# TheProParadox/3dspa_code

Measured on AMD Instinct MI355X. Metric: train-step tracks/sec (B x N_tracks) at T=150, C=772, higher is better.
Workload: dtype bf16

## Files before the change

### 3dspa_code_amd/csrc/rows.hip

```cpp
#include <algorithm>

#include "common.hpp"

namespace SPA_NS {

void k_zero(spa3d_ctx* c, void* p, int64_t bytes) {
  if (c->dry || bytes == 0) return;
  hipError_t e = hipMemsetAsync(p, 0, (size_t)bytes, c->stream);
  if (e != hipSuccess && !c->hip_err) { c->hip_err = (int)e; c->err = std::string("hipMemsetAsync: ") + hipGetErrorString(e); }
}
struct I32x32 { int32_t v[32]; };
__global__ void set_i32_kernel(int32_t* __restrict__ dst, I32x32 a, int n) {
  const int t = threadIdx.x;
#pragma unroll
  for (int i = 0; i < 32; ++i) if (t == i && i < n) dst[i] = a.v[i];
}
void k_set_i32(spa3d_ctx* c, int32_t* dst, const int32_t* host, int64_t n) {
  if (c->dry) return;
  for (int64_t i0 = 0; i0 < n; i0 += 32) {
    I32x32 a; const int m = (int)std::min<int64_t>(32, n - i0);
    for (int i = 0; i < 32; ++i) a.v[i] = i < m ? host[i0 + i] : 0;
    set_i32_kernel<<<1, 64, 0, c->stream>>>(dst + i0, a, m);
  }
  SPA_LAUNCH_CHECK(c);
}
__global__ void mul_kernel(float* __restrict__ a, const float* __restrict__ b, int64_t n) {
  for (int64_t i = (int64_t)blockIdx.x * 256 + threadIdx.x; i < n; i += (int64_t)gridDim.x * 256) a[i] *= b[i];
}
void k_mul(spa3d_ctx* c, float* a, const float* b, int64_t n) {
  if (c->dry || n == 0) return;
  mul_kernel<<<GRID1D(n, 256), 256, 0, c->stream>>>(a, b, n); SPA_LAUNCH_CHECK(c);
}
template <typename T>
__global__ void cast_from_f32_kernel(const float* __restrict__ s, T* __restrict__ d, int64_t n) {
  for (int64_t i = (int64_t)blockIdx.x * 256 + threadIdx.x; i < n; i += (int64_t)gridDim.x * 256) st(d + i, s[i]);
}
template <typename T> void k_cast_from_f32(spa3d_ctx* c, const float* s, T* d, int64_t n) {
  if (c->dry || n == 0) return;
  cast_from_f32_kernel<T><<<GRID1D(n, 256), 256, 0, c->stream>>>(s, d, n); SPA_LAUNCH_CHECK(c);
}
template <typename T>
__global__ void cast_to_f32_kernel(const T* __restrict__ s, float* __restrict__ d, int64_t n) {
  for (int64_t i = (int64_t)blockIdx.x * 256 + threadIdx.x; i < n; i += (int64_t)gridDim.x * 256) d[i] = ld(s + i);
}
template <typename T> void k_cast_to_f32(spa3d_ctx* c, const T* s, float* d, int64_t n) {
  if (c->dry || n == 0) return;
  cast_to_f32_kernel<T><<<GRID1D(n, 256), 256, 0, c->stream>>>(s, d, n); SPA_LAUNCH_CHECK(c);
}
template <typename T>
__global__ void colsum_kernel(const T* __restrict__ x, int64_t rows, int n, int64_t ld_, float* __restrict__ out, int64_t rows_per_block,
                              int rgroup, int rskip, const DetCfg* det) {
  __shared__ float red[4][64];
  const int col = blockIdx.x * 64 + (threadIdx.x & 63), w = threadIdx.x >> 6;
  int64_t r0 = (int64_t)blockIdx.y * rows_per_block, r1 = std::min<int64_t>(rows, r0 + rows_per_block);
  float s = 0.f;
  if (col < n) for (int64_t r = r0 + w; r < r1; r += 4) {
    int64_t pr = r; if (rgroup > 0) pr = r + (r / rgroup + 1) * (int64_t)rskip;
    s += ld(x + pr * ld_ + col);
  }
  red[w][threadIdx.x & 63] = s;
  __syncthreads();
  if (w == 0 && col < n) grad_add(det_read(det), out + col, red[0][threadIdx.x] + red[1][threadIdx.x] + red[2][threadIdx.x] + red[3][threadIdx.x]);
}
template <typename T>
__global__ __launch_bounds__(256) void colsum_vec_kernel(const T* __restrict__ x, int64_t rows, int n, int64_t ld_, float* __restrict__ out,
                                                         int64_t rows_per_block, int rgroup, int rskip, const DetCfg* det) {
  constexpr int NV = VecOf<T>::N;
  __shared__ float red[8][32 * NV];
  const int cx = threadIdx.x & 31, ry = threadIdx.x >> 5;
  const int ch = blockIdx.x * 32 + cx;
  const int64_t r0 = (int64_t)blockIdx.y * rows_per_block, r1 = std::min<int64_t>(rows, r0 + rows_per_block);
  float a[NV];
#pragma unroll
  for (int j = 0; j < NV; ++j) a[j] = 0.f;
  if (ch * NV < n)
    for (int64_t r = r0 + ry; r < r1; r += 8) {
      int64_t pr = r; if (rgroup > 0) pr = r + (r / rgroup + 1) * (int64_t)rskip;
      float v[NV]; load_vec<T, NV>(x + pr * ld_ + ch * NV, v);
#pragma unroll
      for (int j = 0; j < NV; ++j) a[j] += v[j];
    }
#pragma unroll
  for (int j = 0; j < NV; ++j) red[ry][cx * NV + j] = a[j];
  __syncthreads();
  if (ry == 0 && ch * NV < n)
#pragma unroll
    for (int j = 0; j < NV; ++j) {
      float s_ = 0.f;
#pragma unroll
      for (int k = 0; k < 8; ++k) s_ += red[k][cx * NV + j];
      grad_add(det_read(det), out + ch * NV + j, s_);
    }
}
template <typename T>
void k_colsum(spa3d_ctx* c, const T* x, int64_t rows, int n, int64_t ld_, float* out, int rgroup, int rskip) {
  if (c->dry || rows == 0) return;
  constexpr int NV = VecOf<T>::N;
  if (n % NV == 0 && ld_ % NV == 0 && (((uintptr_t)x) & 15) == 0) {
    const int64_t gx = cdiv(n / NV, 32);
    int64_t sp = std::max<int64_t>(1, std::min<int64_t>(cdiv(rows, 64), 2048 / gx + 1));
    int64_t rpb_ = cdiv(rows, sp);
    colsum_vec_kernel<T><<<dim3((unsigned)gx, (unsigned)cdiv(rows, rpb_)), 256, 0, c->stream>>>(x, rows, n, ld_, out, rpb_, rgroup, rskip, c->det);
    SPA_LAUNCH_CHECK(c);
    return;
  }
  int64_t splits = std::max<int64_t>(1, std::min<int64_t>(cdiv(rows, 256), 1024 / std::max<int64_t>(1, cdiv(n, 64)) + 1));
  int64_t rpb = cdiv(rows, splits);
  colsum_kernel<T><<<dim3((unsigned)cdiv(n, 64), (unsigned)cdiv(rows, rpb)), 256, 0, c->stream>>>(x, rows, n, ld_, out, rpb, rgroup, rskip, c->det);
  SPA_LAUNCH_CHECK(c);
}

template <typename T>
__global__ void gather_rows_kernel(const T* __restrict__ src, int64_t srows, T* __restrict__ dst, int64_t n, int d) {
  const int64_t tot = n * d;
  for (int64_t i = (int64_t)blockIdx.x * 256 + threadIdx.x; i < tot; i += (int64_t)gridDim.x * 256) {
    int64_t r = i / d; int j = (int)(i - r * d);
    dst[i] = src[r * srows * d + j];
  }
}
template <typename T> void k_gather_rows(spa3d_ctx* c, const T* src, int64_t srows, T* dst, int64_t n, int d) {
  if (c->dry || n == 0) return;
  gather_rows_kernel<T><<<GRID1D(n * d, 256), 256, 0, c->stream>>>(src, srows, dst, n, d); SPA_LAUNCH_CHECK(c);
}
template <typename T, int MODE>
__global__ void rows_idx_kernel(const T* __restrict__ src, const int32_t* __restrict__ idx, T* __restrict__ dst, int64_t n, int d) {
  constexpr int NV = VecOf<T>::N;
  const int cpr = d / NV;
  const int64_t tot = n * cpr;
  for (int64_t i = (int64_t)blockIdx.x * 256 + threadIdx.x; i < tot; i += (int64_t)gridDim.x * 256) {
    const int64_t r = i / cpr; const int ch = (int)(i - r * cpr);
    const int64_t other = idx[r];
    const int64_t so = (MODE == 0 ? other : r) * d + ch * NV, dofs = (MODE == 0 ? r : other) * d + ch * NV;
    if constexpr (MODE == 2) {
      float a[NV], b[NV];
      load_vec<T, NV>(src + so, a); load_vec<T, NV>(dst + dofs, b);
#pragma unroll
      for (int j = 0; j < NV; ++j) b[j] += a[j];
      store_vec<T, NV>(dst + dofs, b);
    } else {
      *(uint4*)(dst + dofs) = *(const uint4*)(src + so);
    }
  }
}
template <typename T> void k_rows_idx(spa3d_ctx* c, int mode, const T* src, const int32_t* idx, T* dst, int64_t n, int d) {
  if (c->dry || n == 0) return;
  constexpr int NV = VecOf<T>::N;
  if (d % NV) { if (!c->hip_err) { c->hip_err = -5; c->err = "rows_idx: row width must be a multiple of 16 bytes"; } return; }
  const dim3 g = GRID1D(n * (d / NV), 256);
  if (mode == 0) rows_idx_kernel<T, 0><<<g, 256, 0, c->stream>>>(src, idx, dst, n, d);
  else if (mode == 1) rows_idx_kernel<T, 1><<<g, 256, 0, c->stream>>>(src, idx, dst, n, d);
  else rows_idx_kernel<T, 2><<<g, 256, 0, c->stream>>>(src, idx, dst, n, d);
  SPA_LAUNCH_CHECK(c);
}
template <typename T>
__global__ void add_rows_strided_kernel(T* __restrict__ dst, const T* __restrict__ src, int64_t drows, int64_t n, int d) {
  const int64_t tot = n * d;
  for (int64_t i = (int64_t)blockIdx.x * 256 + threadIdx.x; i < tot; i += (int64_t)gridDim.x * 256) {
    int64_t r = i / d; int j = (int)(i - r * d);
    T* p = dst + r * drows * d + j;
    st(p, ld(p) + ld(src + i));
  }
}
template <typename T> void k_add_rows_strided(spa3d_ctx* c, T* dst, const T* src, int64_t drows, int64_t n, int d) {
  if (c->dry || n == 0) return;
  add_rows_strided_kernel<T><<<GRID1D(n * d, 256), 256, 0, c->stream>>>(dst, src, drows, n, d); SPA_LAUNCH_CHECK(c);
}

__global__ __launch_bounds__(256) void prune_count_kernel(const float* __restrict__ km, int64_t nseq, int S, int32_t* __restrict__ cnt) {
  const int lane = threadIdx.x & 63;
  for (int64_t seq = (int64_t)blockIdx.x * 4 + (threadIdx.x >> 6); seq < nseq; seq += (int64_t)gridDim.x * 4) {
    int n = 0;
    for (int t = lane; t < S; t += 64) n += km[seq * S + t] != 0.f ? 1 : 0;
#pragma unroll
    for (int o = 32; o > 0; o >>= 1) n += __shfl_xor(n, o, 64);
    if (lane == 0) cnt[seq] = n;
  }
}
__global__ __launch_bounds__(1024) void prune_scan_kernel(const int32_t* __restrict__ cnt, int64_t n, int32_t* __restrict__ off) {
  __shared__ int32_t part[1024];
  const int tid = threadIdx.x;
  const int64_t per = (n + 1023) / 1024, a = tid * per, b = a + per < n ? a + per : n;
  int32_t s = 0;
  for (int64_t i = a; i < b; ++i) s += cnt[i];
  part[tid] = s;
  __syncthreads();
  for (int o = 1; o < 1024; o <<= 1) {
    const int32_t v = tid >= o ? part[tid - o] : 0;
    __syncthreads();
    part[tid] += v;
    __syncthreads();
  }
  int32_t run = tid ? part[tid - 1] : 0;
  for (int64_t i = a; i < b; ++i) { off[i] = run; run += cnt[i]; }
  if (tid == 1023) off[n] = part[1023];
}
__global__ __launch_bounds__(256) void prune_fill_kernel(const float* __restrict__ km, int64_t nseq, int S, const int32_t* __restrict__ off,
                                                         int32_t* __restrict__ row_src) {
  const int lane = threadIdx.x & 63;
  for (int64_t seq = (int64_t)blockIdx.x * 4 + (threadIdx.x >> 6); seq < nseq; seq += (int64_t)gridDim.x * 4) {
    int base = off[seq];
    for (int t0 = 0; t0 < S; t0 += 64) {
      const int t = t0 + lane;
      const bool keep = t < S && km[seq * S + t] != 0.f;
      const unsigned long long m = __ballot(keep);
      if (keep) row_src[base + __popcll(m & ((1ull << lane) - 1ull))] = (int32_t)(seq * S + t);
      base += __popcll(m);
    }
  }
}
int64_t k_prune_plan(spa3d_ctx* c, const float* km, int64_t nseq, int S, int32_t* cnt, int32_t* seq_off, int32_t* row_src) {
  if (c->dry) return nseq * S;
  prune_count_kernel<<<(unsigned)std::min<int64_t>(cdiv(nseq, 4), 8192), 256, 0, c->stream>>>(km, nseq, S, cnt); SPA_LAUNCH_CHECK(c);
  prune_scan_kernel<<<1, 1024, 0, c->stream>>>(cnt, nseq, seq_off); SPA_LAUNCH_CHECK(c);
  prune_fill_kernel<<<(unsigned)std::min<int64_t>(cdiv(nseq, 4), 8192), 256, 0, c->stream>>>(km, nseq, S, seq_off, row_src); SPA_LAUNCH_CHECK(c);
  int32_t kept = 0;
  if (hipMemcpyAsync(&kept, seq_off + nseq, sizeof(int32_t), hipMemcpyDeviceToHost, c->stream) != hipSuccess ||
      hipStreamSynchronize(c->stream) != hipSuccess) {
    if (!c->hip_err) { c->hip_err = -4; c->err = "prune plan: reading the kept-row count failed"; }
    return nseq * S;
  }
  return kept;
}

__global__ __launch_bounds__(256) void share_plan_kernel(const int32_t* __restrict__ qframe, int Q, int32_t* __restrict__ slot, int32_t* __restrict__ nslot_b,
                                                         int32_t* __restrict__ first_q) {
  extern __shared__ int32_t sh[];
  const int b = blockIdx.x;
  const int32_t* fr = qframe + (int64_t)b * Q;
  for (int q = threadIdx.x; q < Q; q += 256) {
    const int32_t f = fr[q];
    int first = q;
    for (int p = 0; p < q; ++p) if (fr[p] == f) { first = p; break; }
    sh[q] = first;
  }
  __syncthreads();
  if (threadIdx.x == 0) {
    int n = 0;
    for (int q = 0; q < Q; ++q) {
      if (sh[q] == q) { first_q[(int64_t)b * Q + n] = q; sh[q] = -(n + 1); ++n; }
    }
    nslot_b[b] = n;
  }
  __syncthreads();
  for (int q = threadIdx.x; q < Q; q += 256) {
    const int32_t v = sh[q];
    slot[(int64_t)b * Q + q] = v < 0 ? -v - 1 : -sh[v] - 1;
  }
}
__global__ __launch_bounds__(256) void share_plan_finish_kernel(const int32_t* __restrict__ qframe, int B, int Q, int32_t* __restrict__ slot,
                                                                const int32_t* __restrict__ nslot_b, const int32_t* __restrict__ first_q,
                                                                int32_t* __restrict__ slot_b, int32_t* __restrict__ slot_f, int32_t* __restrict__ slot_q0,
                                                                int32_t* __restrict__ total) {
  __shared__ int32_t off[1025];
  if (threadIdx.x == 0) { int a = 0; for (int b = 0; b < B; ++b) { off[b] = a; a += nslot_b[b]; } off[B] = a; total[0] = a; }
  __syncthreads();
  for (int64_t i = threadIdx.x; i < (int64_t)B * Q; i += 256) {
    const int b = (int)(i / Q), j = (int)(i - (int64_t)b * Q);
    slot[i] += off[b];
    if (j < nslot_b[b]) { slot_b[off[b] + j] = b; slot_f[off[b] + j] = qframe[(int64_t)b * Q + first_q[i]]; slot_q0[off[b] + j] = b * Q + first_q[i]; }
  }
}
int64_t k_share_plan(spa3d_ctx* c, const int32_t* qframe, int64_t B, int Q, int32_t* slot, int32_t* slot_b, int32_t* slot_f, int32_t* slot_q0,
                     int32_t* scratch ) {
  if (c->dry) return B * Q;
  if (B > 1024 || Q > 12288) return B * Q;
  int32_t* first_q = scratch; int32_t* nslot_b = scratch + B * Q; int32_t* total = nslot_b + B;
  share_plan_kernel<<<(unsigned)B, 256, Q * sizeof(int32_t), c->stream>>>(qframe, Q, slot, nslot_b, first_q); SPA_LAUNCH_CHECK(c);
  share_plan_finish_kernel<<<1, 256, 0, c->stream>>>(qframe, (int)B, Q, slot, nslot_b, first_q, slot_b, slot_f, slot_q0, total); SPA_LAUNCH_CHECK(c);
  int32_t n = 0;
  if (hipMemcpyAsync(&n, total, sizeof(int32_t), hipMemcpyDeviceToHost, c->stream) != hipSuccess || hipStreamSynchronize(c->stream) != hipSuccess) {
    if (!c->hip_err) { c->hip_err = -4; c->err = "share plan: reading the slot count failed"; }
    return B * Q;
  }
  return n;
}
template <typename T>
__global__ void share_assemble_kernel(const T* __restrict__ qtok, const T* __restrict__ lat, const int32_t* __restrict__ slot_b,
                                      const int32_t* __restrict__ slot_f, int64_t nslot, int64_t BQ, int L, int Cl, int D, T* __restrict__ xU) {
  constexpr int NV = VecOf<T>::N;
  const int cpr = D / NV;
  const int64_t nlat = nslot * L, tot = (nlat + BQ) * cpr;
  for (int64_t i = (int64_t)blockIdx.x * 256 + threadIdx.x; i < tot; i += (int64_t)gridDim.x * 256) {
    const int64_t row = i / cpr; const int j = (int)(i - row * cpr) * NV;
    float v[NV];
    if (row >= nlat) load_vec<T, NV>(qtok + (row - nlat) * D + j, v);
    else {
      const int64_t s_ = row / L; const int n = (int)(row - s_ * L);
      const T* lr = lat + ((int64_t)slot_b[s_] * L + n) * Cl;
      if (j < Cl) load_vec<T, NV>(lr + j, v);
      else {
        const int base = j - Cl + 5 * slot_f[s_];
#pragma unroll
        for (int e = 0; e < NV; ++e) { const int cc = base + e; v[e] = (cc >= 0 && cc < Cl) ? ld(lr + cc) : 0.f; }
      }
    }
    store_vec<T, NV>(xU + row * D + j, v);
  }
}
template <typename T>
void k_share_assemble(spa3d_ctx* c, const T* qtok, const T* lat, const int32_t* slot_b, const int32_t* slot_f, int64_t nslot, int64_t BQ, int L, int Cl,
                      int D, T* xU) {
  if (c->dry || BQ == 0) return;
  constexpr int NV = VecOf<T>::N;
  if (D % NV || Cl % NV) { if (!c->hip_err) { c->hip_err = -5; c->err = "share assemble: widths must be multiples of 16 bytes"; } return; }
  share_assemble_kernel<T><<<GRID1D((nslot * L + BQ) * (D / NV), 256), 256, 0, c->stream>>>(qtok, lat, slot_b, slot_f, nslot, BQ, L, Cl, D, xU);
  SPA_LAUNCH_CHECK(c);
}
template <typename T, bool ADD>
__global__ void share_expand_kernel(const T* __restrict__ src, const int32_t* __restrict__ slot, const int32_t* __restrict__ slot_q0, int64_t nslot,
                                    int64_t nseq, int S, int d, const T* add, T* dst) {
  constexpr int NV = VecOf<T>::N;
  const int cpr = d / NV, L = S - 1;
  const int64_t tot = nseq * S * cpr;
  for (int64_t i = (int64_t)blockIdx.x * 256 + threadIdx.x; i < tot; i += (int64_t)gridDim.x * 256) {
    const int64_t row = i / cpr; const int ch = (int)(i - row * cpr);
    const int64_t seq = row / S; const int tkn = (int)(row - seq * S);
    const int32_t sl = slot[seq];
    const int64_t sr = tkn == 0 ? nslot * L + seq : (int64_t)sl * L + tkn - 1;
    if constexpr (ADD) {
      float b[NV];
      load_vec<T, NV>(add + row * d + ch * NV, b);
      if (tkn == 0 || slot_q0[sl] == (int32_t)seq) {
        float a[NV];
        load_vec<T, NV>(src + sr * d + ch * NV, a);
#pragma unroll
        for (int j = 0; j < NV; ++j) b[j] += a[j];
      }
      store_vec<T, NV>(dst + row * d + ch * NV, b);
    } else {
      *(uint4*)(dst + row * d + ch * NV) = *(const uint4*)(src + sr * d + ch * NV);
    }
  }
}
template <typename T>
void k_share_expand(spa3d_ctx* c, const T* src, const int32_t* slot, const int32_t* slot_q0, int64_t nslot, int64_t nseq, int S, int d, const T* add, T* dst) {
  if (c->dry || nseq == 0) return;
  constexpr int NV = VecOf<T>::N;
  if (d % NV) { if (!c->hip_err) { c->hip_err = -5; c->err = "share expand: row width must be a multiple of 16 bytes"; } return; }
  const dim3 g = GRID1D(nseq * S * (d / NV), 256);
  if (add) share_expand_kernel<T, true><<<g, 256, 0, c->stream>>>(src, slot, slot_q0, nslot, nseq, S, d, add, dst);
  else share_expand_kernel<T, false><<<g, 256, 0, c->stream>>>(src, slot, slot_q0, nslot, nseq, S, d, nullptr, dst);
  SPA_LAUNCH_CHECK(c);
}
template <typename T>
__global__ __launch_bounds__(256) void share_reduce_kernel(const T* __restrict__ src, const int32_t* __restrict__ slot, const int32_t* __restrict__ slot_b,
                                                           int64_t nslot, int Q, int S, int d, T* __restrict__ dstU) {
  constexpr int NV = VecOf<T>::N;
  extern __shared__ int32_t members[];
  __shared__ int32_t wcnt[4], nmem;
  const int64_t s_ = blockIdx.x; const int L = S - 1, cpr = d / NV;
  const int b = slot_b[s_];
  const int lane = threadIdx.x & 63, wv = threadIdx.x >> 6;
  int base = 0;
  for (int q0 = 0; q0 < Q; q0 += 256) {
    const int q = q0 + threadIdx.x;
    const bool mine = q < Q && slot[(int64_t)b * Q + q] == (int32_t)s_;
    const unsigned long long m = __ballot(mine);
    if (lane == 0) wcnt[wv] = __popcll(m);
    __syncthreads();
    int pre = base;
    for (int w2 = 0; w2 < wv; ++w2) pre += wcnt[w2];
    if (mine) members[pre + __popcll(m & ((1ull << lane) - 1ull))] = q;
    base += wcnt[0] + wcnt[1] + wcnt[2] + wcnt[3];
    __syncthreads();
  }
  if (threadIdx.x == 0) nmem = base;
  __syncthreads();
  const int nm = nmem;
  for (int i = threadIdx.x; i < L * cpr; i += 256) {
    const int n = i / cpr, ch = i - n * cpr;
    float acc[NV];
#pragma unroll
    for (int j = 0; j < NV; ++j) acc[j] = 0.f;
    for (int m = 0; m < nm; ++m) {
      float v[NV];
      load_vec<T, NV>(src + (((int64_t)b * Q + members[m]) * S + 1 + n) * d + ch * NV, v);
#pragma unroll
      for (int j = 0; j < NV; ++j) acc[j] += v[j];
    }
    store_vec<T, NV>(dstU + (s_ * L + n) * d + ch * NV, acc);
  }
}
template <typename T>
void k_share_reduce(spa3d_ctx* c, const T* src, const int32_t* slot, const int32_t* slot_b, int64_t nslot, int64_t nseq, int Q, int S, int d, T* dstU) {
  if (c->dry || nseq == 0) return;
  constexpr int NV = VecOf<T>::N;
  if (d % NV) { if (!c->hip_err) { c->hip_err = -5; c->err = "share reduce: row width must be a multiple of 16 bytes"; } return; }
  if (nslot > 0) share_reduce_kernel<T><<<(unsigned)nslot, 256, Q * sizeof(int32_t), c->stream>>>(src, slot, slot_b, nslot, Q, S, d, dstU);
  SPA_LAUNCH_CHECK(c);
  k_gather_rows<T>(c, src, S, dstU + nslot * (S - 1) * d, nseq, d);
}

template <typename T>
__global__ void assemble_kernel(const T* __restrict__ qtok, const T* __restrict__ lat, const int32_t* __restrict__ qframe, int64_t BQ, int Q,
                                int L, int Cl, int D, T* __restrict__ seq) {
  const int64_t tot = BQ * (L + 1) * D;
  for (int64_t i = (int64_t)blockIdx.x * 256 + threadIdx.x; i < tot; i += (int64_t)gridDim.x * 256) {
    int64_t row = i / D; int j = (int)(i - row * D);
    int64_t bq = row / (L + 1); int tkn = (int)(row - bq * (L + 1));
    T v;
    if (tkn == 0) v = qtok[bq * D + j];
    else {
      int64_t b = bq / Q; int n = tkn - 1;
      const T* lr = lat + (b * L + n) * Cl;
      if (j < Cl) v = lr[j];
      else {
        int64_t cc = (int64_t)(j - Cl) + 5 * (int64_t)qframe[bq];
        if (cc >= 0 && cc < Cl) v = lr[cc]; else { T z; st(&z, 0.f); v = z; }
      }
    }
    seq[i] = v;
  }
}
template <typename T>
__global__ void assemble_vec_kernel(const T* __restrict__ qtok, const T* __restrict__ lat, const int32_t* __restrict__ qframe, unsigned nchunk,
                                    int Q, int L, int Cl, int D, T* __restrict__ seq) {
  constexpr int NV = VecOf<T>::N;
  const unsigned cpr = (unsigned)D / NV;
  for (unsigned i = blockIdx.x * 256u + threadIdx.x; i < nchunk; i += gridDim.x * 256u) {
    const unsigned row = i / cpr; const int j = (int)(i - row * cpr) * NV;
    const unsigned bq = row / (unsigned)(L + 1); const int tkn = (int)(row - bq * (unsigned)(L + 1));
    float v[NV];
    if (tkn == 0) load_vec<T, NV>(qtok + (int64_t)bq * D + j, v);
    else {
      const unsigned b = bq / (unsigned)Q;
      const T* lr = lat + ((int64_t)b * L + (tkn - 1)) * Cl;
      if (j < Cl) load_vec<T, NV>(lr + j, v);
      else {
        const int base = j - Cl + 5 * qframe[bq];
#pragma unroll
        for (int e = 0; e < NV; ++e) { const int cc = base + e; v[e] = (cc >= 0 && cc < Cl) ? ld(lr + cc) : 0.f; }
      }
    }
    store_vec<T, NV>(seq + (int64_t)row * D + j, v);
  }
}
template <typename T>
void k_assemble_readout(spa3d_ctx* c, const T* qtok, const T* lat, const int32_t* qframe, int64_t B, int Q, int L, int Cl, int D, T* seq) {
  if (c->dry || B == 0) return;
  constexpr int NV = VecOf<T>::N;
  const int64_t nchunk = B * Q * (L + 1) * (D / NV);
  if (D % NV == 0 && Cl % NV == 0 && nchunk < 0x7fffffffLL && ((((uintptr_t)qtok) | ((uintptr_t)lat) | ((uintptr_t)seq)) & 15) == 0) {
    assemble_vec_kernel<T><<<GRID1D(nchunk, 256), 256, 0, c->stream>>>(qtok, lat, qframe, (unsigned)nchunk, Q, L, Cl, D, seq);
  } else {
    assemble_kernel<T><<<GRID1D(B * Q * (L + 1) * D, 256), 256, 0, c->stream>>>(qtok, lat, qframe, B * Q, Q, L, Cl, D, seq);
  }
  SPA_LAUNCH_CHECK(c);
}
template <typename T, bool ACC>
__global__ void assemble_bwd_lat_kernel(const T* __restrict__ dseq, const int32_t* __restrict__ qframe, int64_t B, int Q, int L, int Cl,
                                        int D, float* __restrict__ dlat) {
  const int64_t tot = B * L * Cl;
  const int Wd = D - Cl;
  for (int64_t i = (int64_t)blockIdx.x * 256 + threadIdx.x; i < tot; i += (int64_t)gridDim.x * 256) {
    int64_t bn = i / Cl; int cc = (int)(i - bn * Cl);
    int64_t b = bn / L; int n = (int)(bn - b * L);
    float s0 = 0.f, s1 = 0.f, s2 = 0.f, s3 = 0.f;
    auto term = [&](int q) {
      const T* r = dseq + (((b * Q + q) * (L + 1)) + 1 + n) * D;
      float t = ld(r + cc);
      const int dd = cc - 5 * qframe[b * Q + q];
      if (dd >= 0 && dd < Wd) t += ld(r + Cl + dd);
      return t;
    };
    int q = 0;
    for (; q + 3 < Q; q += 4) { s0 += term(q); s1 += term(q + 1); s2 += term(q + 2); s3 += term(q + 3); }
    for (; q < Q; ++q) s0 += term(q);
    const float s = (s0 + s1) + (s2 + s3);
    if (ACC) dlat[i] += s; else dlat[i] = s;
  }
}
template <typename T>
void k_assemble_readout_bwd(spa3d_ctx* c, const T* dseq, const int32_t* qframe, int64_t B, int Q, int L, int Cl, int D, T* dqtok,
                            float* dlat, bool accumulate) {
  if (c->dry || B == 0) return;
  k_gather_rows<T>(c, dseq, L + 1, dqtok, B * Q, D);
  if (accumulate) assemble_bwd_lat_kernel<T, true><<<GRID1D(B * L * Cl, 256), 256, 0, c->stream>>>(dseq, qframe, B, Q, L, Cl, D, dlat);
  else assemble_bwd_lat_kernel<T, false><<<GRID1D(B * L * Cl, 256), 256, 0, c->stream>>>(dseq, qframe, B, Q, L, Cl, D, dlat);
  SPA_LAUNCH_CHECK(c);
}

template <typename T>
__global__ void bcast_rows_kernel(const float* __restrict__ src, int64_t per, T* __restrict__ dst, int64_t B) {
  const int64_t tot = per * B;
  for (int64_t i = (int64_t)blockIdx.x * 256 + threadIdx.x; i < tot; i += (int64_t)gridDim.x * 256) st(dst + i, src[i % per]);
}
template <typename T> void k_broadcast_rows(spa3d_ctx* c, const float* src, int rows, int d, T* dst, int64_t B) {
  if (c->dry || B == 0) return;
  bcast_rows_kernel<T><<<GRID1D((int64_t)rows * d * B, 256), 256, 0, c->stream>>>(src, (int64_t)rows * d, dst, B); SPA_LAUNCH_CHECK(c);
}
template <typename T>
__global__ void bcast_grad_kernel(const T* __restrict__ dsrc, int64_t per, int64_t B, int64_t bstride, float* __restrict__ dparam, int64_t bchunk,
                                  const DetCfg* det) {
  const int64_t i = (int64_t)blockIdx.x * 256 + threadIdx.x;
  if (i >= per) return;
  const int64_t b0 = (int64_t)blockIdx.y * bchunk; int64_t b1 = b0 + bchunk; if (b1 > B) b1 = B;
  float s0 = 0.f, s1 = 0.f, s2 = 0.f, s3 = 0.f;
  int64_t b = b0;
  for (; b + 3 < b1; b += 4) {
    s0 += ld(dsrc + b * bstride + i); s1 += ld(dsrc + (b + 1) * bstride + i);
    s2 += ld(dsrc + (b + 2) * bstride + i); s3 += ld(dsrc + (b + 3) * bstride + i);
  }
  for (; b < b1; ++b) s0 += ld(dsrc + b * bstride + i);
  const float s = (s0 + s1) + (s2 + s3);
  if (gridDim.y == 1) dparam[i] += s; else grad_add(det_read(det), dparam + i, s);
}
template <typename T> void k_bcast_grad(spa3d_ctx* c, const T* dsrc, int64_t per, int64_t B, int64_t bstride, float* dparam) {
  if (c->dry || B == 0) return;
  const int64_t gx = cdiv(per, 256);
  int64_t gy = std::max<int64_t>(1, std::min<int64_t>(B / 32, std::max<int64_t>(1, 2048 / gx)));
  const int64_t bchunk = cdiv(B, gy); gy = cdiv(B, bchunk);
  bcast_grad_kernel<T><<<dim3((unsigned)gx, (unsigned)gy), 256, 0, c->stream>>>(dsrc, per, B, bstride, dparam, bchunk, c->det); SPA_LAUNCH_CHECK(c);
}

template <typename T>
__global__ void vis_mean_pool_kernel(const T* __restrict__ tok, const float* __restrict__ vis, int64_t nseq, int T_, int d, T* __restrict__ out) {
  const int64_t tot = nseq * d;
  for (int64_t i = (int64_t)blockIdx.x * 256 + threadIdx.x; i < tot; i += (int64_t)gridDim.x * 256) {
    int64_t s_ = i / d; int j = (int)(i - s_ * d);
    float a = 0.f, cnt = 0.f;
    for (int t = 0; t < T_; ++t) { const float v = vis[s_ * T_ + t] != 0.f ? 1.f : 0.f; a += ld(tok + (s_ * T_ + t) * d + j) * v; cnt += v; }
    st(out + i, a / fmaxf(1.f, cnt));
  }
}
template <typename T> void k_vis_mean_pool(spa3d_ctx* c, const T* tok, const float* vis, int64_t nseq, int T_, int d, T* out) {
  if (c->dry || nseq == 0) return;
  vis_mean_pool_kernel<T><<<GRID1D(nseq * d, 256), 256, 0, c->stream>>>(tok, vis, nseq, T_, d, out); SPA_LAUNCH_CHECK(c);
}
template <typename T>
__global__ void vis_mean_pool_bwd_kernel(const T* __restrict__ dout, const float* __restrict__ vis, int64_t nseq, int T_, int d, T* __restrict__ dtok) {
  const int64_t tot = nseq * T_ * d;
  for (int64_t i = (int64_t)blockIdx.x * 256 + threadIdx.x; i < tot; i += (int64_t)gridDim.x * 256) {
    int64_t r = i / d; int j = (int)(i - r * d);
    int64_t s_ = r / T_;
    float cnt = 0.f;
    for (int t = 0; t < T_; ++t) cnt += vis[s_ * T_ + t] != 0.f ? 1.f : 0.f;
    const float v = vis[r] != 0.f ? 1.f : 0.f;
    st(dtok + i, ld(dout + s_ * d + j) * v / fmaxf(1.f, cnt));
  }
}
template <typename T> void k_vis_mean_pool_bwd(spa3d_ctx* c, const T* dout, const float* vis, int64_t nseq, int T_, int d, T* dtok) {
  if (c->dry || nseq == 0) return;
  vis_mean_pool_bwd_kernel<T><<<GRID1D(nseq * T_ * d, 256), 256, 0, c->stream>>>(dout, vis, nseq, T_, d, dtok); SPA_LAUNCH_CHECK(c);
}

#define INST_ROWS(T) \
  template void k_cast_from_f32<T>(spa3d_ctx*, const float*, T*, int64_t);                                                                 \
  template void k_cast_to_f32<T>(spa3d_ctx*, const T*, float*, int64_t);                                                                   \
  template void k_colsum<T>(spa3d_ctx*, const T*, int64_t, int, int64_t, float*, int, int);                                                \
  template void k_gather_rows<T>(spa3d_ctx*, const T*, int64_t, T*, int64_t, int);                                                         \
  template void k_rows_idx<T>(spa3d_ctx*, int, const T*, const int32_t*, T*, int64_t, int);                                                \
  template void k_add_rows_strided<T>(spa3d_ctx*, T*, const T*, int64_t, int64_t, int);                                                    \
  template void k_share_assemble<T>(spa3d_ctx*, const T*, const T*, const int32_t*, const int32_t*, int64_t, int64_t, int, int, int, T*);  \
  template void k_share_expand<T>(spa3d_ctx*, const T*, const int32_t*, const int32_t*, int64_t, int64_t, int, int, const T*, T*);         \
  template void k_share_reduce<T>(spa3d_ctx*, const T*, const int32_t*, const int32_t*, int64_t, int64_t, int, int, int, T*);              \
  template void k_assemble_readout<T>(spa3d_ctx*, const T*, const T*, const int32_t*, int64_t, int, int, int, int, T*);                    \
  template void k_assemble_readout_bwd<T>(spa3d_ctx*, const T*, const int32_t*, int64_t, int, int, int, int, T*, float*, bool);            \
  template void k_broadcast_rows<T>(spa3d_ctx*, const float*, int, int, T*, int64_t);                                                      \
  template void k_bcast_grad<T>(spa3d_ctx*, const T*, int64_t, int64_t, int64_t, float*);                                                  \
  template void k_vis_mean_pool<T>(spa3d_ctx*, const T*, const float*, int64_t, int, int, T*);                                             \
  template void k_vis_mean_pool_bwd<T>(spa3d_ctx*, const T*, const float*, int64_t, int, int, T*);
INST_ROWS(float)
INST_ROWS(bf16_t)
}
```

Baseline: 92660.

## Restructure share expand/reduce and readout assemble kernels for vectorized row-wise copies

Replaces the per-element share expand with a per-slot kernel that loads each shared latent row once and writes it to every member sequence. It also unrolls the share-reduce accumulation over members and rewrites readout assembly to copy four rows per wave, using nontemporal stores for large outputs. The latent backward becomes one block per (b,n) with vectorized column sums and LDS atomics for the shifted window. These changes target memory bandwidth and index arithmetic in several data-movement kernels, at the cost of more complex code and possible load imbalance when slots have many members.

```diff
diff --git a/3dspa_code_amd/csrc/rows.hip b/3dspa_code_amd/csrc/rows.hip
--- a/3dspa_code_amd/csrc/rows.hip
+++ b/3dspa_code_amd/csrc/rows.hip
@@ -110,6 +110,11 @@
   SPA_LAUNCH_CHECK(c);
 }
 
+typedef unsigned u32x4_t __attribute__((ext_vector_type(4)));
+template <bool NT> __device__ __forceinline__ void store16(void* p, const uint4& v) {
+  if constexpr (NT) { u32x4_t t = {v.x, v.y, v.z, v.w}; __builtin_nontemporal_store(t, (u32x4_t*)p); }
+  else *(uint4*)p = v;
+}
 template <typename T>
 __global__ void gather_rows_kernel(const T* __restrict__ src, int64_t srows, T* __restrict__ dst, int64_t n, int d) {
   const int64_t tot = n * d;
@@ -306,9 +311,9 @@
   share_assemble_kernel<T><<<GRID1D((nslot * L + BQ) * (D / NV), 256), 256, 0, c->stream>>>(qtok, lat, slot_b, slot_f, nslot, BQ, L, Cl, D, xU);
   SPA_LAUNCH_CHECK(c);
 }
-template <typename T, bool ADD>
-__global__ void share_expand_kernel(const T* __restrict__ src, const int32_t* __restrict__ slot, const int32_t* __restrict__ slot_q0, int64_t nslot,
-                                    int64_t nseq, int S, int d, const T* add, T* dst) {
+template <typename T>
+__global__ void share_expand_add_kernel(const T* __restrict__ src, const int32_t* __restrict__ slot, const int32_t* __restrict__ slot_q0, int64_t nslot,
+                                        int64_t nseq, int S, int d, const T* add, T* dst) {
   constexpr int NV = VecOf<T>::N;
   const int cpr = d / NV, L = S - 1;
   const int64_t tot = nseq * S * cpr;
@@ -317,19 +322,62 @@
     const int64_t seq = row / S; const int tkn = (int)(row - seq * S);
     const int32_t sl = slot[seq];
     const int64_t sr = tkn == 0 ? nslot * L + seq : (int64_t)sl * L + tkn - 1;
-    if constexpr (ADD) {
-      float b[NV];
-      load_vec<T, NV>(add + row * d + ch * NV, b);
-      if (tkn == 0 || slot_q0[sl] == (int32_t)seq) {
-        float a[NV];
-        load_vec<T, NV>(src + sr * d + ch * NV, a);
-#pragma unroll
-        for (int j = 0; j < NV; ++j) b[j] += a[j];
+    float b[NV];
+    load_vec<T, NV>(add + row * d + ch * NV, b);
+    if (tkn == 0 || slot_q0[sl] == (int32_t)seq) {
+      float a[NV];
+      load_vec<T, NV>(src + sr * d + ch * NV, a);
+#pragma unroll
+      for (int j = 0; j < NV; ++j) b[j] += a[j];
+    }
+    store_vec<T, NV>(dst + row * d + ch * NV, b);
+  }
+}
+template <typename T>
+__global__ __launch_bounds__(256) void share_expand_slot_kernel(const T* __restrict__ src, const int32_t* __restrict__ slot, const int32_t* __restrict__ slot_q0,
+                                                                int64_t nslot, int64_t nseq, int S, int d, T* __restrict__ dst) {
+  constexpr int NV = VecOf<T>::N, W = 1024;
+  __shared__ int32_t members[W];
+  __shared__ int32_t wcnt[4];
+  const int64_t s_ = blockIdx.x; const int L = S - 1, cpr = d / NV;
+  const int lane = threadIdx.x & 63, wv = threadIdx.x >> 6;
+  const T* srow = src + s_ * L * d;
+  const int64_t nit = (int64_t)L * cpr;
+  for (int64_t c0 = slot_q0[s_]; c0 < nseq; c0 += W) {
+    int nm = 0;
+    for (int r = 0; r < W; r += 256) {
+      const int64_t q = c0 + r + threadIdx.x;
+      const bool mine = q < nseq && slot[q] == (int32_t)s_;
+      const unsigned long long m = __ballot(mine);
+      if (lane == 0) wcnt[wv] = __popcll(m);
+      __syncthreads();
+      int pre = nm;
+      for (int w2 = 0; w2 < wv; ++w2) pre += wcnt[w2];
+      if (mine) members[pre + __popcll(m & ((1ull << lane) - 1ull))] = (int32_t)q;
+      nm += wcnt[0] + wcnt[1] + wcnt[2] + wcnt[3];
+      __syncthreads();
+    }
+    if (nm == 0) continue;
+    int64_t i = threadIdx.x;
+    for (; i + 768 < nit; i += 1024) {
+      uint4 v[4];
+#pragma unroll
+      for (int k = 0; k < 4; ++k) v[k] = *(const uint4*)(srow + (i + k * 256) * NV);
+      for (int m = 0; m < nm; ++m) {
+        T* drow = dst + ((int64_t)members[m] * S + 1) * d;
+#pragma unroll
+        for (int k = 0; k < 4; ++k) *(uint4*)(drow + (i + k * 256) * NV) = v[k];
       }
-      store_vec<T, NV>(dst + row * d + ch * NV, b);
-    } else {
-      *(uint4*)(dst + row * d + ch * NV) = *(const uint4*)(src + sr * d + ch * NV);
-    }
+    }
+    for (; i < nit; i += 256) {
+      const uint4 v = *(const uint4*)(srow + i * NV);
+      for (int m = 0; m < nm; ++m) *(uint4*)(dst + ((int64_t)members[m] * S + 1) * d + i * NV) = v;
+    }
+    for (int t = threadIdx.x; t < nm * cpr; t += 256) {
+      const int m = t / cpr, ch = t - m * cpr; const int64_t seq = members[m];
+      *(uint4*)(dst + seq * S * d + ch * NV) = *(const uint4*)(src + (nslot * L + seq) * d + ch * NV);
+    }
+    __syncthreads();
   }
 }
 template <typename T>
@@ -337,10 +385,43 @@
   if (c->dry || nseq == 0) return;
   constexpr int NV = VecOf<T>::N;
   if (d % NV) { if (!c->hip_err) { c->hip_err = -5; c->err = "share expand: row width must be a multiple of 16 bytes"; } return; }
-  const dim3 g = GRID1D(nseq * S * (d / NV), 256);
-  if (add) share_expand_kernel<T, true><<<g, 256, 0, c->stream>>>(src, slot, slot_q0, nslot, nseq, S, d, add, dst);
-  else share_expand_kernel<T, false><<<g, 256, 0, c->stream>>>(src, slot, slot_q0, nslot, nseq, S, d, nullptr, dst);
+  if (add) share_expand_add_kernel<T><<<GRID1D(nseq * S * (d / NV), 256), 256, 0, c->stream>>>(src, slot, slot_q0, nslot, nseq, S, d, add, dst);
+  else if (nslot > 0) share_expand_slot_kernel<T><<<(unsigned)nslot, 256, 0, c->stream>>>(src, slot, slot_q0, nslot, nseq, S, d, dst);
   SPA_LAUNCH_CHECK(c);
+}
+template <typename T, int K, int NP>
+__device__ __forceinline__ void share_add_rows(const T* const (&p)[NP], const int32_t* mem, int64_t mstride, float (&acc)[NP][VecOf<T>::N]) {
+  constexpr int NV = VecOf<T>::N;
+  float v[NP][K][NV];
+#pragma unroll
+  for (int k = 0; k < K; ++k)
+#pragma unroll
+    for (int r = 0; r < NP; ++r) load_vec<T, NV>(p[r] + mem[k] * mstride, v[r][k]);
+#pragma unroll
+  for (int r = 0; r < NP; ++r)
+#pragma unroll
+    for (int k = 0; k < K; ++k)
+#pragma unroll
+      for (int j = 0; j < NV; ++j) acc[r][j] += v[r][k][j];
+}
+template <typename T, int NP>
+__device__ __forceinline__ void share_reduce_chunks(const T* src0, const int32_t* members, int nm, int64_t mstride, int i, int cpr, int d, T* dst0) {
+  constexpr int NV = VecOf<T>::N;
+  const T* p[NP]; float acc[NP][NV]; int64_t o[NP];
+#pragma unroll
+  for (int r = 0; r < NP; ++r) {
+    const int ii = i + 256 * r, n = ii / cpr, ch = ii - n * cpr;
+    o[r] = (int64_t)n * d + ch * NV; p[r] = src0 + o[r];
+#pragma unroll
+    for (int j = 0; j < NV; ++j) acc[r][j] = 0.f;
+  }
+  int m = 0;
+  for (; m + 3 < nm; m += 4) share_add_rows<T, 4, NP>(p, members + m, mstride, acc);
+  if (nm - m == 3) share_add_rows<T, 3, NP>(p, members + m, mstride, acc);
+  else if (nm - m == 2) share_add_rows<T, 2, NP>(p, members + m, mstride, acc);
+  else if (nm - m == 1) share_add_rows<T, 1, NP>(p, members + m, mstride, acc);
+#pragma unroll
+  for (int r = 0; r < NP; ++r) store_vec<T, NV>(dst0 + o[r], acc[r]);
 }
 template <typename T>
 __global__ __launch_bounds__(256) void share_reduce_kernel(const T* __restrict__ src, const int32_t* __restrict__ slot, const int32_t* __restrict__ slot_b,
@@ -367,19 +448,11 @@
   if (threadIdx.x == 0) nmem = base;
   __syncthreads();
   const int nm = nmem;
-  for (int i = threadIdx.x; i < L * cpr; i += 256) {
-    const int n = i / cpr, ch = i - n * cpr;
-    float acc[NV];
-#pragma unroll
-    for (int j = 0; j < NV; ++j) acc[j] = 0.f;
-    for (int m = 0; m < nm; ++m) {
-      float v[NV];
-      load_vec<T, NV>(src + (((int64_t)b * Q + members[m]) * S + 1 + n) * d + ch * NV, v);
-#pragma unroll
-      for (int j = 0; j < NV; ++j) acc[j] += v[j];
-    }
-    store_vec<T, NV>(dstU + (s_ * L + n) * d + ch * NV, acc);
-  }
+  const T* src0 = src + ((int64_t)b * Q * S + 1) * d;
+  T* dst0 = dstU + s_ * L * d;
+  int i = threadIdx.x;
+  for (; i + 256 < L * cpr; i += 512) share_reduce_chunks<T, 2>(src0, members, nm, (int64_t)S * d, i, cpr, d, dst0);
+  for (; i < L * cpr; i += 256) share_reduce_chunks<T, 1>(src0, members, nm, (int64_t)S * d, i, cpr, d, dst0);
 }
 template <typename T>
 void k_share_reduce(spa3d_ctx* c, const T* src, const int32_t* slot, const int32_t* slot_b, int64_t nslot, int64_t nseq, int Q, int S, int d, T* dstU) {
@@ -412,36 +485,63 @@
     seq[i] = v;
   }
 }
-template <typename T>
-__global__ void assemble_vec_kernel(const T* __restrict__ qtok, const T* __restrict__ lat, const int32_t* __restrict__ qframe, unsigned nchunk,
-                                    int Q, int L, int Cl, int D, T* __restrict__ seq) {
-  constexpr int NV = VecOf<T>::N;
-  const unsigned cpr = (unsigned)D / NV;
-  for (unsigned i = blockIdx.x * 256u + threadIdx.x; i < nchunk; i += gridDim.x * 256u) {
-    const unsigned row = i / cpr; const int j = (int)(i - row * cpr) * NV;
-    const unsigned bq = row / (unsigned)(L + 1); const int tkn = (int)(row - bq * (unsigned)(L + 1));
-    float v[NV];
-    if (tkn == 0) load_vec<T, NV>(qtok + (int64_t)bq * D + j, v);
-    else {
-      const unsigned b = bq / (unsigned)Q;
-      const T* lr = lat + ((int64_t)b * L + (tkn - 1)) * Cl;
-      if (j < Cl) load_vec<T, NV>(lr + j, v);
+template <typename T, bool NT>
+__global__ __launch_bounds__(256) void assemble_rows_kernel(const T* __restrict__ qtok, const T* __restrict__ lat, const int32_t* __restrict__ qframe,
+                                                            int64_t nrows, int Q, int L, int Cl, int D, T* __restrict__ seq) {
+  constexpr int NV = VecOf<T>::N;
+  const int cpr = D / NV, cm = (Cl < D ? Cl : D) / NV, S = L + 1, lane = threadIdx.x & 63;
+  const int wv = __builtin_amdgcn_readfirstlane((int)(threadIdx.x >> 6));
+  const int64_t r0 = ((int64_t)blockIdx.x * 4 + wv) * 4;
+  if (r0 >= nrows) return;
+  const int nr = (int)std::min<int64_t>(4, nrows - r0);
+  int64_t bq = r0 / S; int tkn = (int)(r0 - bq * S);
+  const T* sp[4]; int wb[4]; bool tok0[4];
+#pragma unroll
+  for (int k = 0; k < 4; ++k) {
+    if (k < nr) {
+      tok0[k] = tkn == 0;
+      sp[k] = tok0[k] ? qtok + bq * D : lat + ((bq / Q) * L + (tkn - 1)) * Cl;
+      wb[k] = tok0[k] ? 0 : 5 * qframe[bq];
+      if (++tkn == S) { tkn = 0; ++bq; }
+    } else { sp[k] = sp[0]; wb[k] = wb[0]; tok0[k] = tok0[0]; }
+  }
+  T* dp = seq + r0 * D;
+  if (nr == 4) {
+    for (int ch = lane; ch < cm; ch += 64) {
+      uint4 v[4];
+#pragma unroll
+      for (int k = 0; k < 4; ++k) v[k] = *(const uint4*)(sp[k] + ch * NV);
+#pragma unroll
+      for (int k = 0; k < 4; ++k) store16<NT>(dp + (int64_t)k * D + ch * NV, v[k]);
+    }
+  } else {
+    for (int k = 0; k < nr; ++k)
+      for (int ch = lane; ch < cm; ch += 64) *(uint4*)(dp + (int64_t)k * D + ch * NV) = *(const uint4*)(sp[k] + ch * NV);
+  }
+#pragma unroll
+  for (int k = 0; k < 4; ++k) {
+    if (k >= nr) break;
+    for (int ch = cm + lane; ch < cpr; ch += 64) {
+      T* o = dp + (int64_t)k * D + ch * NV;
+      if (tok0[k]) *(uint4*)o = *(const uint4*)(sp[k] + ch * NV);
       else {
-        const int base = j - Cl + 5 * qframe[bq];
-#pragma unroll
-        for (int e = 0; e < NV; ++e) { const int cc = base + e; v[e] = (cc >= 0 && cc < Cl) ? ld(lr + cc) : 0.f; }
+        const int base = (ch - cm) * NV + wb[k];
+        float v[NV];
+#pragma unroll
+        for (int e = 0; e < NV; ++e) { const int cc = base + e; v[e] = (cc >= 0 && cc < Cl) ? ld(sp[k] + cc) : 0.f; }
+        store_vec<T, NV>(o, v);
       }
     }
-    store_vec<T, NV>(seq + (int64_t)row * D + j, v);
   }
 }
 template <typename T>
 void k_assemble_readout(spa3d_ctx* c, const T* qtok, const T* lat, const int32_t* qframe, int64_t B, int Q, int L, int Cl, int D, T* seq) {
   if (c->dry || B == 0) return;
   constexpr int NV = VecOf<T>::N;
-  const int64_t nchunk = B * Q * (L + 1) * (D / NV);
-  if (D % NV == 0 && Cl % NV == 0 && nchunk < 0x7fffffffLL && ((((uintptr_t)qtok) | ((uintptr_t)lat) | ((uintptr_t)seq)) & 15) == 0) {
-    assemble_vec_kernel<T><<<GRID1D(nchunk, 256), 256, 0, c->stream>>>(qtok, lat, qframe, (unsigned)nchunk, Q, L, Cl, D, seq);
+  const int64_t nrows = B * Q * (L + 1);
+  if (D % NV == 0 && Cl % NV == 0 && nrows / 16 < 0x7fffffffLL && ((((uintptr_t)qtok) | ((uintptr_t)lat) | ((uintptr_t)seq)) & 15) == 0) {
+    if ((double)nrows * D * sizeof(T) >= 512.0 * 1024 * 1024) assemble_rows_kernel<T, true><<<(unsigned)cdiv(nrows, 16), 256, 0, c->stream>>>(qtok, lat, qframe, nrows, Q, L, Cl, D, seq);
+    else assemble_rows_kernel<T, false><<<(unsigned)cdiv(nrows, 16), 256, 0, c->stream>>>(qtok, lat, qframe, nrows, Q, L, Cl, D, seq);
   } else {
     assemble_kernel<T><<<GRID1D(B * Q * (L + 1) * D, 256), 256, 0, c->stream>>>(qtok, lat, qframe, B * Q, Q, L, Cl, D, seq);
   }
@@ -470,12 +570,87 @@
     if (ACC) dlat[i] += s; else dlat[i] = s;
   }
 }
+__device__ __forceinline__ float2 load_pair(const float* p) { return *(const float2*)p; }
+__device__ __forceinline__ float2 load_pair(const bf16_t* p) { const unsigned u = *(const unsigned*)p; return make_float2(unpack_lo(u), unpack_hi(u)); }
+template <typename T, bool ACC>
+__global__ __launch_bounds__(1024) void assemble_bwd_lat_vec_kernel(const T* __restrict__ dseq, const int32_t* __restrict__ qframe, int Q, int L, int Cl,
+                                                                    int D, float* __restrict__ dlat) {
+  constexpr int NV = VecOf<T>::N, U = 8;
+  extern __shared__ float win[];
+  const int64_t bn = blockIdx.x, b = bn / L; const int n = (int)(bn - b * L);
+  const int tid = threadIdx.x, nmain = blockDim.x - 64;
+  for (int i = tid; i < Cl; i += blockDim.x) win[i] = 0.f;
+  __syncthreads();
+  const int64_t qstride = (int64_t)(L + 1) * D;
+  const T* r0 = dseq + (b * Q * (L + 1) + 1 + n) * D;
+  float acc[NV];
+#pragma unroll
+  for (int j = 0; j < NV; ++j) acc[j] = 0.f;
+  if (tid < nmain) {
+    if (tid * NV < Cl) {
+      const T* p = r0 + tid * NV;
+      int q = 0;
+      for (; q + U <= Q; q += U) {
+        float v[U][NV];
+#pragma unroll
+        for (int u = 0; u < U; ++u) load_vec<T, NV>(p + (q + u) * qstride, v[u]);
+#pragma unroll
+        for (int u = 0; u < U; ++u)
+#pragma unroll
+          for (int j = 0; j < NV; ++j) acc[j] += v[u][j];
+      }
+      for (; q < Q; ++q) {
+        float v[NV]; load_vec<T, NV>(p + q * qstride, v);
+#pragma unroll
+        for (int j = 0; j < NV; ++j) acc[j] += v[j];
+      }
+    }
+  } else {
+    const int32_t* fr = qframe + b * Q;
+    const int wpairs = (D - Cl) / 2;
+    for (int w = tid - nmain; w < wpairs; w += 64) {
+      const T* p = r0 + Cl + 2 * w;
+      auto add = [&](int q, const float2 v) {
+        const int c0 = 5 * fr[q] + 2 * w;
+        if (c0 >= 0 && c0 < Cl) atomicAdd(win + c0, v.x);
+        if (c0 + 1 >= 0 && c0 + 1 < Cl) atomicAdd(win + c0 + 1, v.y);
+      };
+      int q = 0;
+      for (; q + U <= Q; q += U) {
+        float2 v[U];
+#pragma unroll
+        for (int u = 0; u < U; ++u) v[u] = load_pair(p + (q + u) * qstride);
+#pragma unroll
+        for (int u = 0; u < U; ++u) add(q + u, v[u]);
+      }
+      for (; q < Q; ++q) add(q, load_pair(p + q * qstride));
+    }
+  }
+  __syncthreads();
+  if (tid < nmain && tid * NV < Cl) {
+    float* o = dlat + bn * Cl + tid * NV;
+#pragma unroll
+    for (int j0 = 0; j0 < NV; j0 += 4) {
+      float4 r = make_float4(acc[j0] + win[tid * NV + j0], acc[j0 + 1] + win[tid * NV + j0 + 1], acc[j0 + 2] + win[tid * NV + j0 + 2],
+                             acc[j0 + 3] + win[tid * NV + j0 + 3]);
+      if (ACC) { const float4 a = *(const float4*)(o + j0); r.x += a.x; r.y += a.y; r.z += a.z; r.w += a.w; }
+      *(float4*)(o + j0) = r;
+    }
+  }
+}
 template <typename T>
 void k_assemble_readout_bwd(spa3d_ctx* c, const T* dseq, const int32_t* qframe, int64_t B, int Q, int L, int Cl, int D, T* dqtok,
                             float* dlat, bool accumulate) {
   if (c->dry || B == 0) return;
   k_gather_rows<T>(c, dseq, L + 1, dqtok, B * Q, D);
-  if (accumulate) assemble_bwd_lat_kernel<T, true><<<GRID1D(B * L * Cl, 256), 256, 0, c->stream>>>(dseq, qframe, B, Q, L, Cl, D, dlat);
+  constexpr int NV = VecOf<T>::N;
+  const int nthr = ((Cl / NV + 63) & ~63) + 64;
+  if (D % NV == 0 && Cl % NV == 0 && Cl <= D && nthr <= 1024 && B * L < 0x7fffffffLL && ((((uintptr_t)dseq) | ((uintptr_t)dlat)) & 15) == 0) {
+    const unsigned g = (unsigned)(B * L); const size_t lds = (size_t)Cl * sizeof(float);
+    if (accumulate) assemble_bwd_lat_vec_kernel<T, true><<<g, nthr, lds, c->stream>>>(dseq, qframe, Q, L, Cl, D, dlat);
+    else assemble_bwd_lat_vec_kernel<T, false><<<g, nthr, lds, c->stream>>>(dseq, qframe, Q, L, Cl, D, dlat);
+  }
+  else if (accumulate) assemble_bwd_lat_kernel<T, true><<<GRID1D(B * L * Cl, 256), 256, 0, c->stream>>>(dseq, qframe, B, Q, L, Cl, D, dlat);
   else assemble_bwd_lat_kernel<T, false><<<GRID1D(B * L * Cl, 256), 256, 0, c->stream>>>(dseq, qframe, B, Q, L, Cl, D, dlat);
   SPA_LAUNCH_CHECK(c);
 }
```

Result: no change. 92930 (median of 6 runs) (+0.3%).
